# argmaxinc/WhisperKit

Measured on NVIDIA H100. Metric: RTFx (audio-sec/s) whisper-large-v3 greedy, higher is better.
Workload: dtype bf16

## Files before the change

whisperkit_b200/csrc/attention_wgmma.cu:

```cuda
#include <stdio.h>
#include <stdlib.h>

#include "common.cuh"
#include "kernels.h"
#include "wgmma.cuh"

namespace wk {

static constexpr int kFaThreads = 384;
static constexpr int kFaBM = 128;
static constexpr int kFaBN = 128;
static constexpr int kFaD = 64;
static constexpr int kFaTile = kFaBN * kFaD * 2;
static constexpr int kFaStages = 4;
static constexpr int kFaSmem = kFaTile  + 2 * kFaStages * kFaTile  + 1024  + 256 ;

struct FaParams {
    int T, H, dm, n_kv_tiles;
    float scale_log2e;
};

__device__ __forceinline__ float fa_ex2(float x) {
    float y;
    asm("ex2.approx.ftz.f32 %0, %1;" : "=f"(y) : "f"(x));
    return y;
}

template <typename T>
__global__ void __launch_bounds__(kFaThreads, 1)
encoder_attention_wgmma_kernel(const __grid_constant__ CUtensorMap tm_qkv, T* __restrict__ out, const FaParams p) {
    extern __shared__ __align__(1024) uint8_t smem_raw[];
    uint8_t* smem = reinterpret_cast<uint8_t*>((reinterpret_cast<uintptr_t>(smem_raw) + 1023) & ~uintptr_t(1023));
    uint8_t* sQ = smem;
    uint8_t* sK = sQ + kFaTile;
    uint8_t* sV = sK + kFaStages * kFaTile;
    uint64_t* bars = reinterpret_cast<uint64_t*>(sV + kFaStages * kFaTile);
    uint64_t* q_full = bars;
    uint64_t* k_full = bars + 1;
    uint64_t* k_empty = k_full + kFaStages;
    uint64_t* v_full = k_empty + kFaStages;
    uint64_t* v_empty = v_full + kFaStages;

    const int warp = threadIdx.x >> 5, lane = threadIdx.x & 31;
    const int bh = blockIdx.y;
    const int b = bh / p.H, h = bh % p.H;
    const int q0 = blockIdx.x * kFaBM;
    const int n = p.n_kv_tiles;

    if (warp == 0 && lane == 0) {
        tma_prefetch_desc(&tm_qkv);
        mbar_init(q_full, 1);
        for (int i = 0; i < kFaStages; ++i) {
            mbar_init(&k_full[i], 1); mbar_init(&k_empty[i], 8);
            mbar_init(&v_full[i], 1); mbar_init(&v_empty[i], 8);
        }
        fence_barrier_init();
    }
    __syncthreads();

    if (warp < 4) {
        asm volatile("setmaxnreg.dec.sync.aligned.u32 40;");
        if (warp == 0 && lane == 0) {
            mbar_expect_tx(q_full, kFaTile);
            tma_load_3d(sQ, &tm_qkv, q_full, h * kFaD, q0, b);
            for (int j = 0; j < n; ++j) {
                const int st = j % kFaStages;
                const uint32_t ph = (j / kFaStages) & 1;
                mbar_wait_bounded(&k_empty[st], ph ^ 1);
                mbar_expect_tx(&k_full[st], kFaTile);
                tma_load_3d(sK + st * kFaTile, &tm_qkv, &k_full[st], p.dm + h * kFaD, j * kFaBN, b);
                mbar_wait_bounded(&v_empty[st], ph ^ 1);
                mbar_expect_tx(&v_full[st], kFaTile);
                tma_load_3d(sV + st * kFaTile, &tm_qkv, &v_full[st], 2 * p.dm + h * kFaD, j * kFaBN, b);
            }
        }
        return;
    }

    asm volatile("setmaxnreg.inc.sync.aligned.u32 232;");
    const int cw = (warp >> 2) - 1;
    const int c_lo = 2 * (lane & 3);
    const float c = p.scale_log2e;
    const uint64_t qd = wgmma_desc_sw128(smem_u32(sQ + cw * 64 * 128));
    float o[32];
#pragma unroll
    for (int i = 0; i < 32; ++i) o[i] = 0.f;
    float m_run[2] = {-INFINITY, -INFINITY}, l_run[2] = {0.f, 0.f};

    mbar_wait_bounded(q_full, 0);
    for (int j = 0; j < n; ++j) {
        const int st = j % kFaStages;
        const uint32_t ph = (j / kFaStages) & 1;
        float s[64];
        mbar_wait_bounded(&k_full[st], ph);
        const uint64_t kd = wgmma_desc_sw128(smem_u32(sK + st * kFaTile));
        wgmma_fence();
#pragma unroll
        for (int k = 0; k < kFaD / 16; ++k) Wgmma<T, 128>::ss(s, qd + (uint64_t)(2 * k), kd + (uint64_t)(2 * k), k > 0 ? 1u : 0u);
        wgmma_commit();
        wgmma_wait<0>();
        __syncwarp();
        if (lane == 0) mbar_arrive(&k_empty[st]);

        const int valid = p.T - j * kFaBN;
        if (valid < kFaBN) {
#pragma unroll
            for (int jj = 0; jj < 16; ++jj)
#pragma unroll
                for (int e = 0; e < 4; ++e)
                    if (8 * jj + c_lo + (e & 1) >= valid) s[4 * jj + e] = -INFINITY;
        }
        uint32_t pa[8][4];
#pragma unroll
        for (int hf = 0; hf < 2; ++hf) {
            float mx = m_run[hf];
#pragma unroll
            for (int jj = 0; jj < 16; ++jj) mx = fmaxf(mx, fmaxf(s[4 * jj + 2 * hf], s[4 * jj + 2 * hf + 1]));
            mx = fmaxf(mx, __shfl_xor_sync(0xffffffffu, mx, 1));
            mx = fmaxf(mx, __shfl_xor_sync(0xffffffffu, mx, 2));
            const float corr = fa_ex2((m_run[hf] - mx) * c);
            m_run[hf] = mx;
            const float nmc = -mx * c;
            float sum = 0.f;
#pragma unroll
            for (int jj = 0; jj < 16; ++jj) {
                const float e0 = fa_ex2(fmaf(s[4 * jj + 2 * hf], c, nmc));
                const float e1 = fa_ex2(fmaf(s[4 * jj + 2 * hf + 1], c, nmc));
                sum += e0 + e1;
                pa[jj >> 1][(jj & 1) * 2 + hf] = T16<T>::pack2(e0, e1);
            }
            l_run[hf] = l_run[hf] * corr + sum;
#pragma unroll
            for (int jj = 0; jj < 8; ++jj) { o[4 * jj + 2 * hf] *= corr; o[4 * jj + 2 * hf + 1] *= corr; }
        }

        mbar_wait_bounded(&v_full[st], ph);
        const uint32_t vs = smem_u32(sV + st * kFaTile);
        wgmma_fence();
#pragma unroll
        for (int kk = 0; kk < kFaBN / 16; ++kk) Wgmma<T, 64>::rs_bt(o, pa[kk], wgmma_desc_sw128(vs + kk * 2048), 1u);
        wgmma_commit();
        wgmma_wait<0>();
        __syncwarp();
        if (lane == 0) mbar_arrive(&v_empty[st]);
    }

#pragma unroll
    for (int hf = 0; hf < 2; ++hf) {
        float l = l_run[hf];
        l += __shfl_xor_sync(0xffffffffu, l, 1);
        l += __shfl_xor_sync(0xffffffffu, l, 2);
        const float inv = 1.f / l;
        const int q = q0 + cw * 64 + (warp & 3) * 16 + (lane >> 2) + 8 * hf;
        if (q >= p.T) continue;
        T* dst = out + ((long long)b * p.T + q) * p.dm + h * kFaD + c_lo;
#pragma unroll
        for (int jj = 0; jj < 8; ++jj)
            *reinterpret_cast<uint32_t*>(dst + 8 * jj) = T16<T>::pack2(o[4 * jj + 2 * hf] * inv, o[4 * jj + 2 * hf + 1] * inv);
    }
}

typedef CUresult (*PFN_encodeTiled)(CUtensorMap*, CUtensorMapDataType, cuuint32_t, void*, const cuuint64_t*, const cuuint64_t*,
                                      const cuuint32_t*, const cuuint32_t*, CUtensorMapInterleave, CUtensorMapSwizzle,
                                      CUtensorMapL2promotion, CUtensorMapFloatOOBfill);

wk_status encoder_attention_wgmma(const void* qkv, void* out, int B, int T, int n_heads, int dtype, cudaStream_t stream) {
    static PFN_encodeTiled enc = nullptr;
    if (!enc) {
        void* fp = nullptr;
        cudaDriverEntryPointQueryResult q;
        if (cudaGetDriverEntryPoint("cuTensorMapEncodeTiled", &fp, cudaEnableDefault, &q) != cudaSuccess || q != cudaDriverEntryPointSuccess) {
            set_error("cuTensorMapEncodeTiled entry point unavailable");
            return WK_ERR_CUDA;
        }
        enc = reinterpret_cast<PFN_encodeTiled>(fp);
    }
    const int dm = n_heads * 64;
    CUtensorMap tm;
    cuuint64_t gdim[3] = {(cuuint64_t)3 * dm, (cuuint64_t)T, (cuuint64_t)B};
    cuuint64_t gstr[2] = {(cuuint64_t)3 * dm * 2, (cuuint64_t)T * 3 * dm * 2};
    cuuint32_t box[3] = {64, 128, 1};
    cuuint32_t es[3] = {1, 1, 1};
    CUresult r = enc(&tm, dtype == WK_DTYPE_F16 ? CU_TENSOR_MAP_DATA_TYPE_FLOAT16 : CU_TENSOR_MAP_DATA_TYPE_BFLOAT16, 3,
                     const_cast<void*>(qkv), gdim, gstr, box, es, CU_TENSOR_MAP_INTERLEAVE_NONE, CU_TENSOR_MAP_SWIZZLE_128B,
                     CU_TENSOR_MAP_L2_PROMOTION_L2_256B, CU_TENSOR_MAP_FLOAT_OOB_FILL_NONE);
    if (r != CUDA_SUCCESS) { set_error("attention tensor map encode failed: %d", (int)r); return WK_ERR_CUDA; }
    FaParams p;
    p.T = T; p.H = n_heads; p.dm = dm;
    p.n_kv_tiles = (T + kFaBN - 1) / kFaBN;
    p.scale_log2e = 0.125f * 1.4426950408889634f;
    dim3 grid((T + kFaBM - 1) / kFaBM, B * n_heads);
    cudaError_t e = cudaSuccess;
    if (dtype == WK_DTYPE_F16) {
        static bool set = false;
        if (!set) { e = cudaFuncSetAttribute(encoder_attention_wgmma_kernel<__half>, cudaFuncAttributeMaxDynamicSharedMemorySize, kFaSmem); set = e == cudaSuccess; }
        if (e == cudaSuccess) encoder_attention_wgmma_kernel<__half><<<grid, kFaThreads, kFaSmem, stream>>>(tm, (__half*)out, p);
    } else {
        static bool set = false;
        if (!set) { e = cudaFuncSetAttribute(encoder_attention_wgmma_kernel<__nv_bfloat16>, cudaFuncAttributeMaxDynamicSharedMemorySize, kFaSmem); set = e == cudaSuccess; }
        if (e == cudaSuccess) encoder_attention_wgmma_kernel<__nv_bfloat16><<<grid, kFaThreads, kFaSmem, stream>>>(tm, (__nv_bfloat16*)out, p);
    }
    if (e != cudaSuccess) { set_error("cudaFuncSetAttribute(fa): %s", cudaGetErrorString(e)); return WK_ERR_CUDA; }
    count_launch();
    e = cudaGetLastError();
    if (e != cudaSuccess) { set_error("encoder_attention_wgmma launch: %s", cudaGetErrorString(e)); return WK_ERR_CUDA; }
    return WK_OK;
}

}
```

Measured before the change: 925.2.

## Make encoder flash attention persistent with three consumer warpgroups and ping-pong scheduling

Turns the encoder attention kernel into a persistent grid sized to the SM count. Three consumer warpgroups cover a 192-row Q block, and Q is double-buffered across work items. Each iteration overlaps the next QK^T wgmma with the current PV wgmma and the softmax, and named barriers rotate MMA issue among the warpgroups. Output goes through shared memory via stmatrix and a TMA store instead of scattered global writes. The aim is more tensor-core overlap and less launch and tail cost, at the price of more complex synchronisation, tighter register budgets (24 producer registers, about 160 per consumer) and more shared memory.

```diff
diff --git a/whisperkit_b200/csrc/attention_wgmma.cu b/whisperkit_b200/csrc/attention_wgmma.cu
--- a/whisperkit_b200/csrc/attention_wgmma.cu
+++ b/whisperkit_b200/csrc/attention_wgmma.cu
@@ -7,16 +7,23 @@
 
 namespace wk {
 
-static constexpr int kFaThreads = 384;
-static constexpr int kFaBM = 128;
+static constexpr int kFaCons = 3;
+static constexpr int kFaThreads = 128 * (1 + kFaCons);
+static constexpr int kFaBM = 64 * kFaCons;
 static constexpr int kFaBN = 128;
 static constexpr int kFaD = 64;
 static constexpr int kFaTile = kFaBN * kFaD * 2;
+static constexpr int kFaQTile = kFaBM * kFaD * 2;
 static constexpr int kFaStages = 4;
-static constexpr int kFaSmem = kFaTile  + 2 * kFaStages * kFaTile  + 1024  + 256 ;
+static constexpr int kFaOutBox = 64 * kFaD * 2;
+static constexpr int kFaSmem = 2 * kFaQTile  + 2 * kFaStages * kFaTile  + kFaCons * kFaOutBox  +
+                               1024  + 256 ;
+static constexpr int kFaProdRegs = 24;
+static constexpr int kFaConsRegs = ((65536 - 128 * kFaProdRegs) / (128 * kFaCons)) / 8 * 8;
+static constexpr int kFaBarSched = 1, kFaBarEpi = 1 + kFaCons;
 
 struct FaParams {
-    int T, H, dm, n_kv_tiles;
+    int T, H, dm, n_kv_tiles, n_qblk, items;
     float scale_log2e;
 };
 
@@ -25,139 +32,226 @@
     asm("ex2.approx.ftz.f32 %0, %1;" : "=f"(y) : "f"(x));
     return y;
 }
+__device__ __forceinline__ void fa_sched_sync(int cw) { asm volatile("bar.sync %0, 256;" ::"r"(kFaBarSched + cw) : "memory"); }
+__device__ __forceinline__ void fa_sched_arrive(int cw) { asm volatile("bar.arrive %0, 256;" ::"r"(kFaBarSched + cw) : "memory"); }
 
 template <typename T>
 __global__ void __launch_bounds__(kFaThreads, 1)
-encoder_attention_wgmma_kernel(const __grid_constant__ CUtensorMap tm_qkv, T* __restrict__ out, const FaParams p) {
+encoder_attention_wgmma_kernel(const __grid_constant__ CUtensorMap tm_qkv, const __grid_constant__ CUtensorMap tm_q,
+                               const __grid_constant__ CUtensorMap tm_out, const FaParams p) {
     extern __shared__ __align__(1024) uint8_t smem_raw[];
     uint8_t* smem = reinterpret_cast<uint8_t*>((reinterpret_cast<uintptr_t>(smem_raw) + 1023) & ~uintptr_t(1023));
     uint8_t* sQ = smem;
-    uint8_t* sK = sQ + kFaTile;
+    uint8_t* sK = sQ + 2 * kFaQTile;
     uint8_t* sV = sK + kFaStages * kFaTile;
-    uint64_t* bars = reinterpret_cast<uint64_t*>(sV + kFaStages * kFaTile);
+    uint8_t* sO = sV + kFaStages * kFaTile;
+    uint64_t* bars = reinterpret_cast<uint64_t*>(sO + kFaCons * kFaOutBox);
     uint64_t* q_full = bars;
-    uint64_t* k_full = bars + 1;
+    uint64_t* q_empty = q_full + 2;
+    uint64_t* k_full = q_empty + 2;
     uint64_t* k_empty = k_full + kFaStages;
     uint64_t* v_full = k_empty + kFaStages;
     uint64_t* v_empty = v_full + kFaStages;
 
     const int warp = threadIdx.x >> 5, lane = threadIdx.x & 31;
-    const int bh = blockIdx.y;
-    const int b = bh / p.H, h = bh % p.H;
-    const int q0 = blockIdx.x * kFaBM;
     const int n = p.n_kv_tiles;
 
     if (warp == 0 && lane == 0) {
         tma_prefetch_desc(&tm_qkv);
-        mbar_init(q_full, 1);
+        tma_prefetch_desc(&tm_q);
+        tma_prefetch_desc(&tm_out);
+        for (int i = 0; i < 2; ++i) { mbar_init(&q_full[i], 1); mbar_init(&q_empty[i], 4 * kFaCons); }
         for (int i = 0; i < kFaStages; ++i) {
-            mbar_init(&k_full[i], 1); mbar_init(&k_empty[i], 8);
-            mbar_init(&v_full[i], 1); mbar_init(&v_empty[i], 8);
+            mbar_init(&k_full[i], 1); mbar_init(&k_empty[i], 4 * kFaCons);
+            mbar_init(&v_full[i], 1); mbar_init(&v_empty[i], 4 * kFaCons);
         }
         fence_barrier_init();
     }
     __syncthreads();
 
     if (warp < 4) {
-        asm volatile("setmaxnreg.dec.sync.aligned.u32 40;");
+        asm volatile("setmaxnreg.dec.sync.aligned.u32 %0;" ::"n"(kFaProdRegs));
         if (warp == 0 && lane == 0) {
-            mbar_expect_tx(q_full, kFaTile);
-            tma_load_3d(sQ, &tm_qkv, q_full, h * kFaD, q0, b);
-            for (int j = 0; j < n; ++j) {
-                const int st = j % kFaStages;
-                const uint32_t ph = (j / kFaStages) & 1;
-                mbar_wait_bounded(&k_empty[st], ph ^ 1);
-                mbar_expect_tx(&k_full[st], kFaTile);
-                tma_load_3d(sK + st * kFaTile, &tm_qkv, &k_full[st], p.dm + h * kFaD, j * kFaBN, b);
-                mbar_wait_bounded(&v_empty[st], ph ^ 1);
-                mbar_expect_tx(&v_full[st], kFaTile);
-                tma_load_3d(sV + st * kFaTile, &tm_qkv, &v_full[st], 2 * p.dm + h * kFaD, j * kFaBN, b);
+            int kv = 0;
+            int it = 0;
+            for (int w = blockIdx.x; w < p.items; w += gridDim.x, ++it) {
+                const int bh = w / p.n_qblk, q0 = (w - bh * p.n_qblk) * kFaBM;
+                const int b = bh / p.H, h = bh - b * p.H;
+                const int qb = it & 1;
+                mbar_wait(&q_empty[qb], ((it >> 1) & 1) ^ 1);
+                mbar_expect_tx(&q_full[qb], kFaQTile);
+                tma_load_3d(sQ + qb * kFaQTile, &tm_q, &q_full[qb], h * kFaD, q0, b);
+                for (int j = 0; j < n; ++j, ++kv) {
+                    const int st = kv % kFaStages;
+                    const uint32_t ph = (kv / kFaStages) & 1;
+                    mbar_wait(&k_empty[st], ph ^ 1);
+                    mbar_expect_tx(&k_full[st], kFaTile);
+                    tma_load_3d(sK + st * kFaTile, &tm_qkv, &k_full[st], p.dm + h * kFaD, j * kFaBN, b);
+                    mbar_wait(&v_empty[st], ph ^ 1);
+                    mbar_expect_tx(&v_full[st], kFaTile);
+                    tma_load_3d(sV + st * kFaTile, &tm_qkv, &v_full[st], 2 * p.dm + h * kFaD, j * kFaBN, b);
+                }
             }
         }
         return;
     }
 
-    asm volatile("setmaxnreg.inc.sync.aligned.u32 232;");
+    asm volatile("setmaxnreg.inc.sync.aligned.u32 %0;" ::"n"(kFaConsRegs));
     const int cw = (warp >> 2) - 1;
+    const int wg_tid = threadIdx.x & 127;
     const int c_lo = 2 * (lane & 3);
     const float c = p.scale_log2e;
-    const uint64_t qd = wgmma_desc_sw128(smem_u32(sQ + cw * 64 * 128));
-    float o[32];
-#pragma unroll
-    for (int i = 0; i < 32; ++i) o[i] = 0.f;
-    float m_run[2] = {-INFINITY, -INFINITY}, l_run[2] = {0.f, 0.f};
-
-    mbar_wait_bounded(q_full, 0);
-    for (int j = 0; j < n; ++j) {
-        const int st = j % kFaStages;
-        const uint32_t ph = (j / kFaStages) & 1;
+    uint8_t* my_out = sO + cw * kFaOutBox;
+    const int mrow = 16 * (wg_tid >> 5) + 8 * ((lane >> 3) & 1) + (lane & 7);
+    const int mj = lane >> 4;
+
+    if (cw == kFaCons - 1) fa_sched_arrive(0);
+    int kv = 0;
+    int it = 0;
+    for (int w = blockIdx.x; w < p.items; w += gridDim.x, ++it) {
+        const int bh = w / p.n_qblk, q0 = (w - bh * p.n_qblk) * kFaBM;
+        const int b = bh / p.H, h = bh - b * p.H;
+        const int qb = it & 1;
+        const bool last_item = w + (int)gridDim.x >= p.items;
+        auto hand_over = [&](int j) {
+            if (!(cw == kFaCons - 1 && last_item && j == n - 1)) fa_sched_arrive(cw + 1 == kFaCons ? 0 : cw + 1);
+        };
+        const uint64_t qd = wgmma_desc_sw128(smem_u32(sQ + qb * kFaQTile + cw * 64 * 128));
+        float o[32];
+#pragma unroll
+        for (int i = 0; i < 32; ++i) o[i] = 0.f;
+        float m_run[2] = {-INFINITY, -INFINITY}, l_run[2] = {0.f, 0.f};
+        float corr[2];
         float s[64];
-        mbar_wait_bounded(&k_full[st], ph);
-        const uint64_t kd = wgmma_desc_sw128(smem_u32(sK + st * kFaTile));
-        wgmma_fence();
-#pragma unroll
-        for (int k = 0; k < kFaD / 16; ++k) Wgmma<T, 128>::ss(s, qd + (uint64_t)(2 * k), kd + (uint64_t)(2 * k), k > 0 ? 1u : 0u);
-        wgmma_commit();
+        uint32_t pa[8][4];
+
+        auto issue_s = [&](int st) {
+            const uint64_t kd = wgmma_desc_sw128(smem_u32(sK + st * kFaTile));
+            wgmma_fence();
+#pragma unroll
+            for (int k = 0; k < kFaD / 16; ++k) Wgmma<T, 128>::ss(s, qd + (uint64_t)(2 * k), kd + (uint64_t)(2 * k), k > 0 ? 1u : 0u);
+            wgmma_commit();
+        };
+        auto issue_pv = [&](int st) {
+#pragma unroll
+            for (int hf = 0; hf < 2; ++hf)
+#pragma unroll
+                for (int jj = 0; jj < 8; ++jj) { o[4 * jj + 2 * hf] *= corr[hf]; o[4 * jj + 2 * hf + 1] *= corr[hf]; }
+            const uint32_t vs = smem_u32(sV + st * kFaTile);
+            wgmma_fence();
+#pragma unroll
+            for (int kk = 0; kk < kFaBN / 16; ++kk) Wgmma<T, 64>::rs_bt(o, pa[kk], wgmma_desc_sw128(vs + kk * 2048), 1u);
+            wgmma_commit();
+        };
+        auto softmax = [&](int j) {
+            const int valid = p.T - j * kFaBN;
+            if (valid < kFaBN) {
+#pragma unroll
+                for (int jj = 0; jj < 16; ++jj)
+#pragma unroll
+                    for (int e = 0; e < 4; ++e)
+                        if (8 * jj + c_lo + (e & 1) >= valid) s[4 * jj + e] = -INFINITY;
+            }
+#pragma unroll
+            for (int hf = 0; hf < 2; ++hf) {
+                float mx = m_run[hf];
+#pragma unroll
+                for (int jj = 0; jj < 16; ++jj) mx = fmaxf(mx, fmaxf(s[4 * jj + 2 * hf], s[4 * jj + 2 * hf + 1]));
+                mx = fmaxf(mx, __shfl_xor_sync(0xffffffffu, mx, 1));
+                mx = fmaxf(mx, __shfl_xor_sync(0xffffffffu, mx, 2));
+                corr[hf] = fa_ex2((m_run[hf] - mx) * c);
+                m_run[hf] = mx;
+                const float nmc = -mx * c;
+                float sum = 0.f;
+#pragma unroll
+                for (int jj = 0; jj < 16; ++jj) {
+                    const float e0 = fa_ex2(fmaf(s[4 * jj + 2 * hf], c, nmc));
+                    const float e1 = fa_ex2(fmaf(s[4 * jj + 2 * hf + 1], c, nmc));
+                    sum += e0 + e1;
+                    s[4 * jj + 2 * hf] = e0;
+                    s[4 * jj + 2 * hf + 1] = e1;
+                }
+                l_run[hf] = l_run[hf] * corr[hf] + sum;
+            }
+        };
+        auto pack_p = [&]() {
+#pragma unroll
+            for (int jj = 0; jj < 16; ++jj)
+#pragma unroll
+                for (int hf = 0; hf < 2; ++hf) pa[jj >> 1][(jj & 1) * 2 + hf] = T16<T>::pack2(s[4 * jj + 2 * hf], s[4 * jj + 2 * hf + 1]);
+        };
+        auto release = [&](uint64_t* bar) {
+            __syncwarp();
+            if (lane == 0) mbar_arrive(bar);
+        };
+
+        mbar_wait(&q_full[qb], (it >> 1) & 1);
+        int st_prev = kv % kFaStages;
+        uint32_t ph_prev = (kv / kFaStages) & 1;
+        mbar_wait(&k_full[st_prev], ph_prev);
+        fa_sched_sync(cw);
+        issue_s(st_prev);
+        hand_over(0);
         wgmma_wait<0>();
-        __syncwarp();
-        if (lane == 0) mbar_arrive(&k_empty[st]);
-
-        const int valid = p.T - j * kFaBN;
-        if (valid < kFaBN) {
-#pragma unroll
-            for (int jj = 0; jj < 16; ++jj)
-#pragma unroll
-                for (int e = 0; e < 4; ++e)
-                    if (8 * jj + c_lo + (e & 1) >= valid) s[4 * jj + e] = -INFINITY;
-        }
-        uint32_t pa[8][4];
+        release(&k_empty[st_prev]);
+        softmax(0);
+        pack_p();
+        ++kv;
+        for (int j = 1; j < n; ++j, ++kv) {
+            const int st = kv % kFaStages;
+            const uint32_t ph = (kv / kFaStages) & 1;
+            mbar_wait(&k_full[st], ph);
+            mbar_wait(&v_full[st_prev], ph_prev);
+            fa_sched_sync(cw);
+            issue_s(st);
+            issue_pv(st_prev);
+            hand_over(j);
+            wgmma_wait<1>();
+            release(&k_empty[st]);
+            softmax(j);
+            wgmma_wait<0>();
+            release(&v_empty[st_prev]);
+            pack_p();
+            st_prev = st;
+            ph_prev = ph;
+        }
+        mbar_wait(&v_full[st_prev], ph_prev);
+        issue_pv(st_prev);
+        wgmma_wait<0>();
+        release(&v_empty[st_prev]);
+        release(&q_empty[qb]);
+
+        if (wg_tid == 0) bulk_wait_read_all();
+        warpgroup_bar(kFaBarEpi + cw);
+        float inv[2];
 #pragma unroll
         for (int hf = 0; hf < 2; ++hf) {
-            float mx = m_run[hf];
-#pragma unroll
-            for (int jj = 0; jj < 16; ++jj) mx = fmaxf(mx, fmaxf(s[4 * jj + 2 * hf], s[4 * jj + 2 * hf + 1]));
-            mx = fmaxf(mx, __shfl_xor_sync(0xffffffffu, mx, 1));
-            mx = fmaxf(mx, __shfl_xor_sync(0xffffffffu, mx, 2));
-            const float corr = fa_ex2((m_run[hf] - mx) * c);
-            m_run[hf] = mx;
-            const float nmc = -mx * c;
-            float sum = 0.f;
-#pragma unroll
-            for (int jj = 0; jj < 16; ++jj) {
-                const float e0 = fa_ex2(fmaf(s[4 * jj + 2 * hf], c, nmc));
-                const float e1 = fa_ex2(fmaf(s[4 * jj + 2 * hf + 1], c, nmc));
-                sum += e0 + e1;
-                pa[jj >> 1][(jj & 1) * 2 + hf] = T16<T>::pack2(e0, e1);
+            float l = l_run[hf];
+            l += __shfl_xor_sync(0xffffffffu, l, 1);
+            l += __shfl_xor_sync(0xffffffffu, l, 2);
+            inv[hf] = 1.f / l;
+        }
+        const uint32_t sb = smem_u32(my_out);
+#pragma unroll
+        for (int jp = 0; jp < 4; ++jp) {
+            uint32_t r[4];
+#pragma unroll
+            for (int hj = 0; hj < 2; ++hj) {
+                const int jj = 2 * jp + hj;
+                r[2 * hj] = T16<T>::pack2(o[4 * jj] * inv[0], o[4 * jj + 1] * inv[0]);
+                r[2 * hj + 1] = T16<T>::pack2(o[4 * jj + 2] * inv[1], o[4 * jj + 3] * inv[1]);
             }
-            l_run[hf] = l_run[hf] * corr + sum;
-#pragma unroll
-            for (int jj = 0; jj < 8; ++jj) { o[4 * jj + 2 * hf] *= corr; o[4 * jj + 2 * hf + 1] *= corr; }
-        }
-
-        mbar_wait_bounded(&v_full[st], ph);
-        const uint32_t vs = smem_u32(sV + st * kFaTile);
-        wgmma_fence();
-#pragma unroll
-        for (int kk = 0; kk < kFaBN / 16; ++kk) Wgmma<T, 64>::rs_bt(o, pa[kk], wgmma_desc_sw128(vs + kk * 2048), 1u);
-        wgmma_commit();
-        wgmma_wait<0>();
-        __syncwarp();
-        if (lane == 0) mbar_arrive(&v_empty[st]);
-    }
-
-#pragma unroll
-    for (int hf = 0; hf < 2; ++hf) {
-        float l = l_run[hf];
-        l += __shfl_xor_sync(0xffffffffu, l, 1);
-        l += __shfl_xor_sync(0xffffffffu, l, 2);
-        const float inv = 1.f / l;
-        const int q = q0 + cw * 64 + (warp & 3) * 16 + (lane >> 2) + 8 * hf;
-        if (q >= p.T) continue;
-        T* dst = out + ((long long)b * p.T + q) * p.dm + h * kFaD + c_lo;
-#pragma unroll
-        for (int jj = 0; jj < 8; ++jj)
-            *reinterpret_cast<uint32_t*>(dst + 8 * jj) = T16<T>::pack2(o[4 * jj + 2 * hf] * inv, o[4 * jj + 2 * hf + 1] * inv);
-    }
+            stmatrix_x4(sb + (uint32_t)(mrow * 128 + (((2 * jp + mj) ^ (mrow & 7)) << 4)), r[0], r[1], r[2], r[3]);
+        }
+        fence_proxy_async();
+        warpgroup_bar(kFaBarEpi + cw);
+        const int row0 = q0 + cw * 64;
+        if (wg_tid == 0 && row0 < p.T) {
+            tma_store_3d(&tm_out, my_out, h * kFaD, row0, b);
+            bulk_commit();
+        }
+    }
+    if (wg_tid == 0) bulk_wait_all();
 }
 
 typedef CUresult (*PFN_encodeTiled)(CUtensorMap*, CUtensorMapDataType, cuuint32_t, void*, const cuuint64_t*, const cuuint64_t*,
@@ -176,29 +270,45 @@
         enc = reinterpret_cast<PFN_encodeTiled>(fp);
     }
     const int dm = n_heads * 64;
-    CUtensorMap tm;
-    cuuint64_t gdim[3] = {(cuuint64_t)3 * dm, (cuuint64_t)T, (cuuint64_t)B};
-    cuuint64_t gstr[2] = {(cuuint64_t)3 * dm * 2, (cuuint64_t)T * 3 * dm * 2};
-    cuuint32_t box[3] = {64, 128, 1};
-    cuuint32_t es[3] = {1, 1, 1};
-    CUresult r = enc(&tm, dtype == WK_DTYPE_F16 ? CU_TENSOR_MAP_DATA_TYPE_FLOAT16 : CU_TENSOR_MAP_DATA_TYPE_BFLOAT16, 3,
-                     const_cast<void*>(qkv), gdim, gstr, box, es, CU_TENSOR_MAP_INTERLEAVE_NONE, CU_TENSOR_MAP_SWIZZLE_128B,
-                     CU_TENSOR_MAP_L2_PROMOTION_L2_256B, CU_TENSOR_MAP_FLOAT_OOB_FILL_NONE);
-    if (r != CUDA_SUCCESS) { set_error("attention tensor map encode failed: %d", (int)r); return WK_ERR_CUDA; }
+    const CUtensorMapDataType tdt = dtype == WK_DTYPE_F16 ? CU_TENSOR_MAP_DATA_TYPE_FLOAT16 : CU_TENSOR_MAP_DATA_TYPE_BFLOAT16;
+    CUtensorMap tm, tm_q, tm_out;
+    for (int i = 0; i < 2; ++i) {
+        cuuint64_t gdim[3] = {(cuuint64_t)3 * dm, (cuuint64_t)T, (cuuint64_t)B};
+        cuuint64_t gstr[2] = {(cuuint64_t)3 * dm * 2, (cuuint64_t)T * 3 * dm * 2};
+        cuuint32_t box[3] = {64, (cuuint32_t)(i == 0 ? kFaBN : kFaBM), 1};
+        cuuint32_t es[3] = {1, 1, 1};
+        CUresult r = enc(i == 0 ? &tm : &tm_q, tdt, 3, const_cast<void*>(qkv), gdim, gstr, box, es, CU_TENSOR_MAP_INTERLEAVE_NONE,
+                         CU_TENSOR_MAP_SWIZZLE_128B, CU_TENSOR_MAP_L2_PROMOTION_L2_256B, CU_TENSOR_MAP_FLOAT_OOB_FILL_NONE);
+        if (r != CUDA_SUCCESS) { set_error("attention tensor map encode failed: %d", (int)r); return WK_ERR_CUDA; }
+    }
+    {
+        cuuint64_t gdim[3] = {(cuuint64_t)dm, (cuuint64_t)T, (cuuint64_t)B};
+        cuuint64_t gstr[2] = {(cuuint64_t)dm * 2, (cuuint64_t)T * dm * 2};
+        cuuint32_t box[3] = {64, 64, 1};
+        cuuint32_t es[3] = {1, 1, 1};
+        CUresult r = enc(&tm_out, tdt, 3, out, gdim, gstr, box, es, CU_TENSOR_MAP_INTERLEAVE_NONE, CU_TENSOR_MAP_SWIZZLE_128B,
+                         CU_TENSOR_MAP_L2_PROMOTION_NONE, CU_TENSOR_MAP_FLOAT_OOB_FILL_NONE);
+        if (r != CUDA_SUCCESS) { set_error("attention output tensor map encode failed: %d", (int)r); return WK_ERR_CUDA; }
+    }
+    int dev = 0, sms = 0;
+    cudaError_t e = cudaGetDevice(&dev);
+    if (e == cudaSuccess) e = cudaDeviceGetAttribute(&sms, cudaDevAttrMultiProcessorCount, dev);
+    if (e != cudaSuccess) { set_error("encoder_attention_wgmma: %s", cudaGetErrorString(e)); return WK_ERR_CUDA; }
     FaParams p;
     p.T = T; p.H = n_heads; p.dm = dm;
     p.n_kv_tiles = (T + kFaBN - 1) / kFaBN;
+    p.n_qblk = (T + kFaBM - 1) / kFaBM;
+    p.items = B * n_heads * p.n_qblk;
     p.scale_log2e = 0.125f * 1.4426950408889634f;
-    dim3 grid((T + kFaBM - 1) / kFaBM, B * n_heads);
-    cudaError_t e = cudaSuccess;
+    const dim3 grid(p.items < sms ? p.items : sms);
     if (dtype == WK_DTYPE_F16) {
         static bool set = false;
         if (!set) { e = cudaFuncSetAttribute(encoder_attention_wgmma_kernel<__half>, cudaFuncAttributeMaxDynamicSharedMemorySize, kFaSmem); set = e == cudaSuccess; }
-        if (e == cudaSuccess) encoder_attention_wgmma_kernel<__half><<<grid, kFaThreads, kFaSmem, stream>>>(tm, (__half*)out, p);
+        if (e == cudaSuccess) encoder_attention_wgmma_kernel<__half><<<grid, kFaThreads, kFaSmem, stream>>>(tm, tm_q, tm_out, p);
     } else {
         static bool set = false;
         if (!set) { e = cudaFuncSetAttribute(encoder_attention_wgmma_kernel<__nv_bfloat16>, cudaFuncAttributeMaxDynamicSharedMemorySize, kFaSmem); set = e == cudaSuccess; }
-        if (e == cudaSuccess) encoder_attention_wgmma_kernel<__nv_bfloat16><<<grid, kFaThreads, kFaSmem, stream>>>(tm, (__nv_bfloat16*)out, p);
+        if (e == cudaSuccess) encoder_attention_wgmma_kernel<__nv_bfloat16><<<grid, kFaThreads, kFaSmem, stream>>>(tm, tm_q, tm_out, p);
     }
     if (e != cudaSuccess) { set_error("cudaFuncSetAttribute(fa): %s", cudaGetErrorString(e)); return WK_ERR_CUDA; }
     count_launch();
```

Result: faster. 936.7 (median of 6 runs) (+1.2%).
